# cedricrommel/manipose

Measured on AMD Instinct MI355X. Metric: train poses/sec (whole node), H36M T=243 J=17 K=5, higher is better.
Workload: dtype bf16x3; 1 GPU; H36M lifting T=243 J=17 K=5 ManiPose full (C=512, depth 8), train step fwd+WTA loss+bwd+allreduce+Adam; windows_per_gpu=158, global_batch=158, seq_len=243, parallelism=dp1, precision=bf16x3, gradient_exchange=none

## Files before the change

### manipose_amd/csrc/attention_mfma.hip

```cpp
#include <stdlib.h>
#include "common.h"
#include "kernels.h"

namespace mp {

typedef short bf16x8_t __attribute__((ext_vector_type(8)));
typedef short bf16x4_t __attribute__((ext_vector_type(4)));
typedef float f32x4 __attribute__((ext_vector_type(4)));

constexpr int TP = 256;
constexpr int NTILE = TP / 16;

__device__ __forceinline__ float sfma(float a, float b, float c) { return __builtin_fmaf(a, b, c); }
__device__ __forceinline__ float sadd(float a, float b) {
#pragma clang fp contract(off)
  return a + b;
}
__device__ __forceinline__ float smul(float a, float b) {
#pragma clang fp contract(off)
  return a * b;
}
__device__ __forceinline__ float ssub(float a, float b) {
#pragma clang fp contract(off)
  return a - b;
}

__device__ __forceinline__ float4 bf16x4_to_float4(const uint2& r) {
  return make_float4(__uint_as_float(r.x << 16), __uint_as_float(r.x & 0xffff0000u), __uint_as_float(r.y << 16), __uint_as_float(r.y & 0xffff0000u));
}

template <int D> struct ACfg {
  static constexpr int ROWB = D == 64 ? 128 : 2 * D + 16;
  static __device__ __forceinline__ int swz(int row) { return D == 64 ? (row & 7) : 0; }
  static constexpr int KS = (D + 31) / 32;
  static constexpr int DB = D / 16;
  static constexpr int CH = D / 8;
};

template <int D, int NIMG>
__device__ __forceinline__ void stage_rows_multi(char* const (&S)[NIMG], const bf16* const (&base)[NIMG], const long (&stride)[NIMG], int T, int rows,
                                                 int tid, int nthreads) {
  constexpr int CH = ACfg<D>::CH, ROWB = ACfg<D>::ROWB, U = 2;
  const int total = rows * CH;
  for (int idx0 = tid; idx0 < total; idx0 += U * nthreads) {
    uint4 x[NIMG][U];
#pragma unroll
    for (int u = 0; u < U; ++u) {
      const int idx = min(idx0 + u * nthreads, total - 1);
      const int t = idx / CH, c = idx - t * CH, tc = min(t, T - 1);
#pragma unroll
      for (int im = 0; im < NIMG; ++im) x[im][u] = *reinterpret_cast<const uint4*>(base[im] + (long)tc * stride[im] + c * 8);
    }
#pragma unroll
    for (int u = 0; u < U; ++u) {
      const int idx = idx0 + u * nthreads;
      const int t = idx / CH, c = idx - t * CH;
      if (idx < total) {
#pragma unroll
        for (int im = 0; im < NIMG; ++im)
          *reinterpret_cast<uint4*>(S[im] + t * ROWB + ((c ^ ACfg<D>::swz(t)) << 4)) = (t < T) ? x[im][u] : make_uint4(0u, 0u, 0u, 0u);
      }
    }
  }
}

template <int D> struct ImgRd {
  int fr[ACfg<D>::KS], tc[ACfg<D>::DB];
  bool zero;
  __device__ __forceinline__ void init(const char* img, int lane) {
    constexpr int ROWB = ACfg<D>::ROWB;
    typedef const __attribute__((address_space(3))) char* lds_cptr;
    const int img_off = (int)(unsigned)(size_t)((lds_cptr)img);
    const int l15 = lane & 15, g = lane >> 4, q = l15 >> 2, p = l15 & 3;
    zero = D < 32 && 8 * g >= D;
#pragma unroll
    for (int ks = 0; ks < ACfg<D>::KS; ++ks) {
      fr[ks] = img_off + l15 * ROWB + (((4 * ks + g) ^ ACfg<D>::swz(l15)) << 4);
      asm volatile("" : "+v"(fr[ks]));
    }
#pragma unroll
    for (int db = 0; db < ACfg<D>::DB; ++db) {
      const int row = 4 * g + q;
      tc[db] = img_off + row * ROWB + (((2 * db + (p >> 1)) ^ ACfg<D>::swz(row)) << 4) + (p & 1) * 8;
      asm volatile("" : "+v"(tc[db]));
    }
// ... 731 lines not shown
    if (next < nunits && !MP_ADBG(1)) fetch(next);
    first_unit = false;
    bool q_fetched = false;
    const int h = unit % H, bj = unit / H, j = bj % J, b = bj / J;
#pragma unroll
    for (int sidx = 0; sidx < 2; ++sidx) {
      const int qt = wave + sidx * nw;
      if (qt >= ntile) break;
      const int tq = qt * 16 + l15;
      f32x4 s[NTILE];
      float mx = -INFINITY;
#pragma unroll
      for (int kt = 0; kt < NTILE; ++kt) {
        f32x4 acc = {0.f, 0.f, 0.f, 0.f};
        if (kt < ntile) {
#pragma unroll
          for (int ks = 0; ks < KS; ++ks) {
            const int krow = MP_ADBG(2) ? 0 : kt * 16;
            const bf16x8_t kh = Khr.rows(ks, krow), kl = Khr.rows(ks, krow, dlo);
            if (MP_ADBG(8)) { acc[0] += __builtin_bit_cast(float, (int)kh[0] + (int)kl[1]); continue; }
            MP_MFMA3(acc, kh, kl, qn_h[sidx][ks], qn_l[sidx][ks]);
          }
#pragma unroll
          for (int r = 0; r < 4; ++r) acc[r] = smul(acc[r], scale2);
          if (kt == ntile - 1) {
#pragma unroll
            for (int r = 0; r < 4; ++r)
              if (kt * 16 + 4 * g + r >= T) acc[r] = -INFINITY;
          }
          mx = fmaxf(fmaxf(mx, fmaxf(acc[0], acc[1])), fmaxf(acc[2], acc[3]));
        } else {
          acc = f32x4{-INFINITY, -INFINITY, -INFINITY, -INFINITY};
        }
        s[kt] = acc;
      }
      if (sidx == 1 && next < nunits) { fetch_q(next); q_fetched = true; }
      mx = group_max(mx);
      float sum = 0.f;
#pragma unroll
      for (int kt = 0; kt < NTILE; ++kt) {
        if (MP_ADBG(4)) { sum += s[kt][0]; continue; }
        if (kt < ntile) {
          f32x4 e;
#pragma unroll
          for (int r = 0; r < 4; ++r) e[r] = __builtin_amdgcn_exp2f(ssub(s[kt][r], mx));
          s[kt] = e;
          sum += (e[0] + e[1]) + (e[2] + e[3]);
        } else {
          s[kt] = f32x4{0.f, 0.f, 0.f, 0.f};
        }
      }
      sum = group_sum(sum);
      f32x4 o[DB];
#pragma unroll
      for (int db = 0; db < DB; ++db) o[db] = f32x4{0.f, 0.f, 0.f, 0.f};
#pragma unroll
      for (int kp = 0; kp < NTILE / 2; ++kp) {
        if (2 * kp < ntile) {
          bf16x8_t bph, bpl;
          pack_acc_x2(s[2 * kp], s[2 * kp + 1], bph, bpl);
#pragma unroll
          for (int db = 0; db < DB; ++db) {
            const int vrow = MP_ADBG(2) ? 0 : kp * 32;
            const bf16x8_t vh = Vhr.cols(db, vrow), vl = Vhr.cols(db, vrow, dlo);
            if (MP_ADBG(8)) { o[db][0] += __builtin_bit_cast(float, (int)vh[0] + (int)vl[1] + (int)bph[0] + (int)bpl[0]); continue; }
            MP_MFMA3(o[db], vh, vl, bph, bpl);
          }
        }
      }
      if (tq < T && !(MP_ADBG(16) && sum != 12345.f)) {
        const float inv = 1.0f / sum;
        const long oo = ((long)(b * T + tq) * J + j) * C + h * D;
#pragma unroll
        for (int db = 0; db < DB; ++db) store4_o<F8O>(out_hi + oo + 16 * db + 4 * g, out_lo + oo + 16 * db + 4 * g, o[db], inv);
        if (g == 0) lse[(long)unit * T + tq] = (mx + __log2f(sum)) * 0.6931471805599453f;
      }
    }
    if (next >= nunits) break;
    if (!q_fetched) fetch_q(next);
    unit = next;
  }
}

__device__ __forceinline__ void tm_dma_region(char* __restrict__ region, const bf16* __restrict__ p_hi, const bf16* __restrict__ p_lo, long rs3, int T,
                                              int rows, int lane, int wave, int nw) {
  typedef __attribute__((address_space(3))) void* lptr;
  typedef const __attribute__((address_space(1))) void* gptr;
  const int per_img = rows >> 3;
  for (int n = wave; n < 2 * per_img; n += nw) {
    const int img = n >= per_img, q = n - img * per_img;
    const int r = q * 8 + (lane >> 3), c = (lane & 7) ^ (r & 7);
    const bf16* src = (img ? p_lo : p_hi) + (long)min(r, T - 1) * rs3 + c * 8;
    __builtin_amdgcn_global_load_lds((gptr)src, (lptr)(region + n * 1024), 16, 0, 0);
  }
}

template <bool FULL, bool F8O = false>
__global__ __launch_bounds__(512) void attn_tmfma_fwd_x3p_kernel(const bf16* __restrict__ qkv_hi, const bf16* __restrict__ qkv_lo,
                                                                  bf16* __restrict__ out_hi, bf16* __restrict__ out_lo,
                                                                  float* __restrict__ lse, int nunits, int T, int J, int C, int H, float scale) {
#pragma clang fp contract(off)
  extern __shared__ __attribute__((aligned(16))) char sm[];
  constexpr int D = 64, ROWB = 128, KS = 2, DB = 4, NW = 8, OPITCH = 144;
  const int rows = FULL ? TP : (T + 31) & ~31;
  const int tid = threadIdx.x, lane = tid & 63, g = lane >> 4, l15 = lane & 15;
  const int wave = __builtin_amdgcn_readfirstlane(tid >> 6);
  const long rs3 = (long)J * 3 * C;
  const int ntile = FULL ? NTILE : (T + 15) >> 4;
  const int img_bytes = rows * ROWB;
  char* const regA = sm;
  char* const regB = sm + 2 * img_bytes;
  char* const obuf = sm + 4 * img_bytes + wave * (16 * OPITCH);
  ImgRd<D> Khr, Vhr;
  Khr.init(regA, lane);
  Vhr.init(regB, lane);
  const int dlo = __builtin_amdgcn_readfirstlane(img_bytes);
  const float scale2 = scale * 1.4426950408889634f;
  auto unit_base = [&](int unit) -> long {
    const int h = unit % H, bj = unit / H, j = bj % J, b = bj / J;
    return ((long)b * T * J + j) * 3 * C + h * D;
  };
  bf16x8_t qh[2][KS], ql[2][KS];
  auto fetch_q = [&](int unit) {
    const long qoff = unit_base(unit);
#pragma unroll
    for (int sidx = 0; sidx < 2; ++sidx) {
      const int tq = min((wave + sidx * NW) * 16 + l15, T - 1);
#pragma unroll
      for (int ks = 0; ks < KS; ++ks) {
        qh[sidx][ks] = *reinterpret_cast<const bf16x8_t*>(qkv_hi + qoff + (long)tq * rs3 + 32 * ks + 8 * g);
        ql[sidx][ks] = *reinterpret_cast<const bf16x8_t*>(qkv_lo + qoff + (long)tq * rs3 + 32 * ks + 8 * g);
      }
    }
  };
  int unit = blockIdx.x;
  if (unit >= nunits) return;
  {
    const long qoff = unit_base(unit);
    tm_dma_region(regA, qkv_hi + qoff + C, qkv_lo + qoff + C, rs3, T, rows, lane, wave, NW);
  }
  fetch_q(unit);
  const bool two = wave + NW < ntile;
  while (true) {
    const long qoff = unit_base(unit);
    const int h = unit % H, bj = unit / H, j = bj % J, b = bj / J;
    __builtin_amdgcn_s_waitcnt(0x0070);
    __builtin_amdgcn_s_barrier();
    tm_dma_region(regB, qkv_hi + qoff + 2 * C, qkv_lo + qoff + 2 * C, rs3, T, rows, lane, wave, NW);
    f32x4 s[2][NTILE];
    float mx[2] = {-INFINITY, -INFINITY};
#pragma unroll
    for (int kt = 0; kt < NTILE; ++kt) {
      f32x4 a0 = {0.f, 0.f, 0.f, 0.f}, a1 = {0.f, 0.f, 0.f, 0.f};
      if (kt < ntile) {
#pragma unroll
        for (int ks = 0; ks < KS; ++ks) {
          const bf16x8_t kh = Khr.rows(ks, kt * 16), kl = Khr.rows(ks, kt * 16, dlo);
          MP_MFMA3(a0, kh, kl, qh[0][ks], ql[0][ks]);
          MP_MFMA3(a1, kh, kl, qh[1][ks], ql[1][ks]);
        }
#pragma unroll
        for (int r = 0; r < 4; ++r) { a0[r] = smul(a0[r], scale2); a1[r] = smul(a1[r], scale2); }
        if (kt == ntile - 1) {
#pragma unroll
          for (int r = 0; r < 4; ++r)
            if (kt * 16 + 4 * g + r >= T) { a0[r] = -INFINITY; a1[r] = -INFINITY; }
        }
        mx[0] = fmaxf(fmaxf(mx[0], fmaxf(a0[0], a0[1])), fmaxf(a0[2], a0[3]));
        mx[1] = fmaxf(fmaxf(mx[1], fmaxf(a1[0], a1[1])), fmaxf(a1[2], a1[3]));
      } else {
        a0 = f32x4{-INFINITY, -INFINITY, -INFINITY, -INFINITY};
        a1 = a0;
      }
      s[0][kt] = a0;
      s[1][kt] = a1;
    }
    float sum[2];
#pragma unroll
    for (int sidx = 0; sidx < 2; ++sidx) {
      mx[sidx] = group_max(mx[sidx]);
      float sm_ = 0.f;
#pragma unroll
      for (int kt = 0; kt < NTILE; ++kt) {
        if (kt < ntile) {
          f32x4 e;
#pragma unroll
          for (int r = 0; r < 4; ++r) e[r] = __builtin_amdgcn_exp2f(ssub(s[sidx][kt][r], mx[sidx]));
          s[sidx][kt] = e;
          sm_ += (e[0] + e[1]) + (e[2] + e[3]);
        } else {
          s[sidx][kt] = f32x4{0.f, 0.f, 0.f, 0.f};
        }
      }
      sum[sidx] = group_sum(sm_);
    }
    __builtin_amdgcn_s_waitcnt(0x0070);
    __builtin_amdgcn_s_barrier();
    const int next = unit + gridDim.x;
    if (next < nunits) {
      const long noff = unit_base(next);
      tm_dma_region(regA, qkv_hi + noff + C, qkv_lo + noff + C, rs3, T, rows, lane, wave, NW);
      fetch_q(next);
    }
    f32x4 o[2][DB];
#pragma unroll
    for (int sidx = 0; sidx < 2; ++sidx)
#pragma unroll
      for (int db = 0; db < DB; ++db) o[sidx][db] = f32x4{0.f, 0.f, 0.f, 0.f};
#pragma unroll
    for (int kp = 0; kp < NTILE / 2; ++kp) {
      if (2 * kp < ntile) {
        bf16x8_t p0h, p0l, p1h, p1l;
        pack_acc_x2(s[0][2 * kp], s[0][2 * kp + 1], p0h, p0l);
        pack_acc_x2(s[1][2 * kp], s[1][2 * kp + 1], p1h, p1l);
#pragma unroll
        for (int db = 0; db < DB; ++db) {
          const bf16x8_t vh = Vhr.cols(db, kp * 32), vl = Vhr.cols(db, kp * 32, dlo);
          MP_MFMA3(o[0][db], vh, vl, p0h, p0l);
          MP_MFMA3(o[1][db], vh, vl, p1h, p1l);
        }
      }
    }
#pragma unroll
    for (int sidx = 0; sidx < 2; ++sidx) {
      if (sidx == 1 && !two) break;
      const int qt = wave + sidx * NW;
      const float inv = 1.0f / sum[sidx];
      uint2 hv[DB], lv[DB];
#pragma unroll
      for (int db = 0; db < DB; ++db) {
        if constexpr (F8O) pack4_f16f8(make_float4(o[sidx][db][0] * inv, o[sidx][db][1] * inv, o[sidx][db][2] * inv, o[sidx][db][3] * inv), hv[db], lv[db]);
        else {
          split_bf16x2(o[sidx][db][0] * inv, o[sidx][db][1] * inv, hv[db].x, lv[db].x);
          split_bf16x2(o[sidx][db][2] * inv, o[sidx][db][3] * inv, hv[db].y, lv[db].y);
        }
      }
#pragma unroll
      for (int plane = 0; plane < 2; ++plane) {
#pragma unroll
        for (int db = 0; db < DB; ++db) *reinterpret_cast<uint2*>(obuf + l15 * OPITCH + 32 * db + 8 * g) = plane ? lv[db] : hv[db];
        bf16* const dst = plane ? out_lo : out_hi;
#pragma unroll
        for (int pass = 0; pass < 2; ++pass) {
          const int row = pass * 8 + (lane >> 3), tq = qt * 16 + row;
          const uint4 v = *reinterpret_cast<const uint4*>(obuf + row * OPITCH + (lane & 7) * 16);
          if (tq < T) *reinterpret_cast<uint4*>(dst + ((long)(b * T + tq) * J + j) * C + h * D + (lane & 7) * 8) = v;
        }
      }
      const int tq = qt * 16 + l15;
      if (g == 0 && tq < T) lse[(long)unit * T + tq] = (mx[sidx] + __log2f(sum[sidx])) * 0.6931471805599453f;
    }
    if (next >= nunits) break;
    unit = next;
  }
}

static int g_attn_two_phase = 1;
void attn_two_phase(int on) { g_attn_two_phase = on; }

template <int D, bool F8O = false>
__global__ __launch_bounds__(512) void attn_smfma_fwd_x3_kernel(const bf16* __restrict__ qkv_hi, const bf16* __restrict__ qkv_lo,
                                                                 bf16* __restrict__ out_hi, bf16* __restrict__ out_lo, int nframes, int N, int C,
                                                                 int H, float scale) {
  extern __shared__ __attribute__((aligned(16))) char sm[];
  constexpr int KS = ACfg<D>::KS, DB = ACfg<D>::DB, PER = 7;
  const int tid = threadIdx.x, lane = tid & 63, h = __builtin_amdgcn_readfirstlane(tid >> 6), nthreads = (int)blockDim.x;
  const int g = lane >> 4, l15 = lane & 15;
  const int pitch = 6 * C + 16, cpr = (6 * C) >> 4, nchunk = N * cpr;
  char* sh = sm;
  char* sl = sm + N * pitch;
  uint4 pre[2][PER];
  auto fetch = [&](int f) {
    const char* bh = reinterpret_cast<const char*>(qkv_hi + (long)f * N * 3 * C);
    const char* bl = reinterpret_cast<const char*>(qkv_lo + (long)f * N * 3 * C);
#pragma unroll
    for (int i = 0; i < PER; ++i) {
      const int idx = tid + i * nthreads;
      uint4 a = make_uint4(0u, 0u, 0u, 0u), c = a;
      if (idx < nchunk) { a = *reinterpret_cast<const uint4*>(bh + (long)idx * 16); c = *reinterpret_cast<const uint4*>(bl + (long)idx * 16); }
      pre[0][i] = a; pre[1][i] = c;
    }
  };
  auto commit = [&]() {
#pragma unroll
    for (int i = 0; i < PER; ++i) {
      const int idx = tid + i * nthreads, r = idx / cpr, k = idx - r * cpr;
      if (idx < nchunk) {
        *reinterpret_cast<uint4*>(sh + r * pitch + k * 16) = pre[0][i];
        *reinterpret_cast<uint4*>(sl + r * pitch + k * 16) = pre[1][i];
      }
    }
  };
  const int oq = h * D * 2, ok = 2 * C + oq, ov = 4 * C + oq;
  int f = blockIdx.x;
  if (f >= nframes) return;
  fetch(f);
  while (true) {
    __syncthreads();
    commit();
    __syncthreads();
    const int next = f + gridDim.x;
    if (next < nframes) fetch(next);
    bf16x8_t kfh[2][KS], kfl[2][KS];
#pragma unroll
    for (int t = 0; t < 2; ++t)
#pragma unroll
      for (int ks = 0; ks < KS; ++ks) {
        kfh[t][ks] = frag_tok<D>(sh, pitch, ok, 16 * t, ks, lane, N);
        kfl[t][ks] = frag_tok<D>(sl, pitch, ok, 16 * t, ks, lane, N);
      }
    bf16x8_t vTh[DB], vTl[DB];
#pragma unroll
    for (int db = 0; db < DB; ++db) {
      vTh[db] = frag_tokT<D>(sh, pitch, ov, db, lane, N);
      vTl[db] = frag_tokT<D>(sl, pitch, ov, db, lane, N);
    }
#pragma unroll
    for (int qt = 0; qt < 2; ++qt) {
      if (qt * 16 >= N) break;
      bf16x8_t qfh[KS], qfl[KS];
#pragma unroll
      for (int ks = 0; ks < KS; ++ks) {
        qfh[ks] = frag_tok<D>(sh, pitch, oq, 16 * qt, ks, lane, N);
        qfl[ks] = frag_tok<D>(sl, pitch, oq, 16 * qt, ks, lane, N);
      }
      f32x4 s0 = {0.f, 0.f, 0.f, 0.f}, s1 = {0.f, 0.f, 0.f, 0.f};
#pragma unroll
      for (int ks = 0; ks < KS; ++ks) {
        MP_MFMA3(s0, kfh[0][ks], kfl[0][ks], qfh[ks], qfl[ks]);
        MP_MFMA3(s1, kfh[1][ks], kfl[1][ks], qfh[ks], qfl[ks]);
      }
      col_softmax(s0, s1, g, N, scale);
      bf16x8_t bph, bpl;
      pack_acc_x2(s0, s1, bph, bpl);
      const int tq = qt * 16 + l15;
#pragma unroll
      for (int db = 0; db < DB; ++db) {
        f32x4 o = {0.f, 0.f, 0.f, 0.f};
        MP_MFMA3(o, vTh[db], vTl[db], bph, bpl);
        if (tq < N) {
          const long oo = ((long)f * N + tq) * C + h * D + 16 * db + 4 * g;
          store4_o<F8O>(out_hi + oo, out_lo + oo, o, 1.0f);
// ... 148 lines not shown
      MP_HIP(hipFuncSetAttribute((const void*)attn_tmfma_fwd_x3p_kernel<true>, hipFuncAttributeMaxDynamicSharedMemorySize, (int)(4 * TP * 128 + 8 * 16 * 144)));
      MP_HIP(hipFuncSetAttribute((const void*)attn_tmfma_fwd_x3p_kernel<false, true>, hipFuncAttributeMaxDynamicSharedMemorySize, (int)(4 * TP * 128 + 8 * 16 * 144)));
      MP_HIP(hipFuncSetAttribute((const void*)attn_tmfma_fwd_x3p_kernel<true, true>, hipFuncAttributeMaxDynamicSharedMemorySize, (int)(4 * TP * 128 + 8 * 16 * 144)));
      attr_set = true;
    }
    const int grid = min(units, num_cus());
    const bool full = ((T + 15) >> 4) == NTILE ATTN_X3P_FULL_GUARD;
    if (out_f16f8) {
      if (full) hipLaunchKernelGGL((attn_tmfma_fwd_x3p_kernel<true, true>), dim3(grid), dim3(512), lds, st, qkv_hi, qkv_lo, out_hi, out_lo, lse, units, T, J, C, H, scale);
      else hipLaunchKernelGGL((attn_tmfma_fwd_x3p_kernel<false, true>), dim3(grid), dim3(512), lds, st, qkv_hi, qkv_lo, out_hi, out_lo, lse, units, T, J, C, H, scale);
    } else if (full)
      hipLaunchKernelGGL(attn_tmfma_fwd_x3p_kernel<true>, dim3(grid), dim3(512), lds, st, qkv_hi, qkv_lo, out_hi, out_lo, lse, units, T, J, C, H, scale);
    else
      hipLaunchKernelGGL(attn_tmfma_fwd_x3p_kernel<false>, dim3(grid), dim3(512), lds, st, qkv_hi, qkv_lo, out_hi, out_lo, lse, units, T, J, C, H, scale);
    MP_LAUNCH_CHECK();
    return MP_OK;
  }
  if (D == 64 && out_f16f8) return launch_tmfma_fwd_x3<64, true>(qkv_hi, qkv_lo, out_hi, out_lo, lse, units, T, J, C, H, scale, st);
  if (D == 64) return launch_tmfma_fwd_x3<64>(qkv_hi, qkv_lo, out_hi, out_lo, lse, units, T, J, C, H, scale, st);
  return launch_tmfma_fwd_x3<16>(qkv_hi, qkv_lo, out_hi, out_lo, lse, units, T, J, C, H, scale, st);
}

bool attn_tmfma_supported(int T, int D) { return T <= TP && (D == 64 || D == 16); }

template <int D, int NTC>
static int launch_tmfma_fwd(const bf16* qkv, bf16* out, float* lse, int units, int T, int J, int C, int H, float scale, hipStream_t st) {
  const int ntile = (T + 15) >> 4;
  const int waves = NTC ? 8 : (ntile <= 8 ? (ntile + 1) / 2 : 8);
  const int rows = NTC ? TP : (T + 31) & ~31;
  const size_t lds = 2 * (size_t)rows * ACfg<D>::ROWB;
  static bool attr_set = false;
  if (!attr_set) {
    MP_HIP(hipFuncSetAttribute((const void*)attn_tmfma_fwd_kernel<D, NTC>, hipFuncAttributeMaxDynamicSharedMemorySize,
                               (int)(2 * TP * ACfg<D>::ROWB)));
    attr_set = true;
  }
  hipLaunchKernelGGL((attn_tmfma_fwd_kernel<D, NTC>), dim3(units), dim3(64 * waves), lds, st, qkv, out, lse, T, J, C, H, scale);
  MP_LAUNCH_CHECK();
  return MP_OK;
}
int attn_tmfma_fwd(const bf16* qkv, bf16* out, float* lse, int B, int T, int J, int C, int H, hipStream_t st) {
  const int D = C / H;
  MP_CHECK(attn_tmfma_supported(T, D) && C % 8 == 0, MP_ERR_ARG, "attn_tmfma_fwd: T=%d D=%d unsupported", T, D);
  const float scale = attn_qk_scale(D);
  const int units = B * J * H;
  if (D == 64) return launch_tmfma_fwd<64, 0>(qkv, out, lse, units, T, J, C, H, scale, st);
  return launch_tmfma_fwd<16, 0>(qkv, out, lse, units, T, J, C, H, scale, st);
}

template <int D, int NTC>
static int launch_tmfma_bwd(const bf16* qkv, const bf16* out, const bf16* dout, const float* lse, bf16* dqkv, int units, int T, int J, int C,
                            int H, float scale, int dbg, hipStream_t st, int out_f16) {
  const int ntile = (T + 15) >> 4;
  const int waves = NTC ? 16 : ((ntile >= 5 && ntile <= 7) ? 4 : min(16, ntile));
  const int rows = NTC ? TP : (T + 31) & ~31;
  const size_t lds = 4 * (size_t)rows * ACfg<D>::ROWB + 2 * rows * sizeof(float);
  static bool attr_set = false;
  if (!attr_set) {
    MP_HIP(hipFuncSetAttribute((const void*)attn_tmfma_bwd_kernel<D, NTC, false>, hipFuncAttributeMaxDynamicSharedMemorySize,
                               (int)(4 * TP * ACfg<D>::ROWB + 2 * TP * sizeof(float))));
    MP_HIP(hipFuncSetAttribute((const void*)attn_tmfma_bwd_kernel<D, NTC, true>, hipFuncAttributeMaxDynamicSharedMemorySize,
                               (int)(4 * TP * ACfg<D>::ROWB + 2 * TP * sizeof(float))));
    attr_set = true;
  }
  if (g_grad_f16 != nullptr)
    hipLaunchKernelGGL((attn_tmfma_bwd_kernel<D, NTC, true>), dim3(units), dim3(64 * waves), lds, st, qkv, out, dout, lse, dqkv, T, J, C, H, scale, dbg, g_grad_f16, out_f16);
  else
    hipLaunchKernelGGL((attn_tmfma_bwd_kernel<D, NTC, false>), dim3(units), dim3(64 * waves), lds, st, qkv, out, dout, lse, dqkv, T, J, C, H, scale, dbg, g_grad_f16, out_f16);
  MP_LAUNCH_CHECK();
  return MP_OK;
}
int attn_tmfma_bwd(const bf16* qkv, const bf16* out, const bf16* dout, const float* lse, bf16* dqkv, int B, int T, int J, int C, int H,
                   hipStream_t st, int out_f16) {
  const int D = C / H;
  MP_CHECK(attn_tmfma_supported(T, D) && C % 8 == 0, MP_ERR_ARG, "attn_tmfma_bwd: T=%d D=%d unsupported", T, D);
  const float scale = attn_qk_scale(D);
  const int units = B * J * H;
#ifdef MP_GEMM_DIAG
  static const int dbg = [] { const char* e = getenv("MANIPOSE_ATTN_DEBUG"); return e ? atoi(e) : 0; }();
#else
  constexpr int dbg = 0;
#endif
  const bool full = T > 240;
  if (D == 64) return full ? launch_tmfma_bwd<64, 16>(qkv, out, dout, lse, dqkv, units, T, J, C, H, scale, dbg, st, out_f16)
                           : launch_tmfma_bwd<64, 0>(qkv, out, dout, lse, dqkv, units, T, J, C, H, scale, dbg, st, out_f16);
  return full ? launch_tmfma_bwd<16, 16>(qkv, out, dout, lse, dqkv, units, T, J, C, H, scale, dbg, st, out_f16)
              : launch_tmfma_bwd<16, 0>(qkv, out, dout, lse, dqkv, units, T, J, C, H, scale, dbg, st, out_f16);
}

}
```

### manipose_amd/csrc/capi.hip

```cpp
#include <string.h>
#include "common.h"
#include "kernels.h"
#include "../../include/manipose_hip.h"

namespace mp {
const char* last_error();
long wgrad_f32_slab_floats(int Mtok, int Nout, int Kin);
bool attn_tmfma_supported(int T, int D);
bool attn_smfma_supported(int N, int D, int H);
}
using namespace mp;

static LossCfg to_cfg(const mp_loss_config* c) {
  LossCfg l;
  l.beta = c->rmcl_score_reg; l.vel_w = c->vel_loss; l.smooth_w = c->smooth_reg; l.use_joint_weights = c->w_loss; l.squared = c->sq_loss;
  for (int j = 0; j < 17; ++j) l.joint_weights[j] = c->joint_weights[j];
  return l;
}

extern "C" {

int mp_abi_version(void) { return MP_ABI_VERSION; }
const char* mp_last_error(void) { return mp::last_error(); }

// ... 468 lines not shown
  return ingest_pose2d(raw, raw_joints, raw_channels, frames, (long)N, joint_map, J, res_w, res_h, out, (hipStream_t)stream);
}

int mp_procrustes_errors(const float* pred, const float* gt, const uint8_t* mask, int64_t N, int J, float pred_scale, float gt_scale,
                         float pck_threshold, float auc_max, int auc_steps, float* out, float* scratch, int64_t scratch_floats, void* stream) {
  return procrustes_errors(pred, gt, mask, (long)N, J, pred_scale, gt_scale, pck_threshold, auc_max, auc_steps, 1, out, scratch,
                           (long)scratch_floats, (hipStream_t)stream);
}

int mp_pose_metrics_row_floats(void) { return pose_metrics_row_floats(); }
int mp_bone_length_table(const float* pred, const int64_t* pred_strides, const float* gt, const int64_t* gt_strides, int B, int L, int signed_diff,
                         float* out, void* stream) {
  MP_CHECK(pred && pred_strides && gt && gt_strides && out, MP_ERR_ARG, "mp_bone_length_table: null pointer");
  long ps[4], gs[4];
  for (int i = 0; i < 4; ++i) { ps[i] = (long)pred_strides[i]; gs[i] = (long)gt_strides[i]; }
  return bone_length_table(pred, ps, gt, gs, B, L, signed_diff, out, (hipStream_t)stream);
}
int mp_pose_metrics(const float* pred, const int64_t* pred_strides, const float* gt, const int64_t* gt_strides, const uint8_t* mask, int B,
                    int L, int J, float pred_scale, float gt_scale, float pck_threshold, float auc_max, int auc_steps, int scale_align,
                    float* out, float* len0, float* scratch, int64_t scratch_floats, void* stream) {
  MP_CHECK(pred && pred_strides && out && len0 && scratch, MP_ERR_ARG, "mp_pose_metrics: null pointer");
  long ps[4], gs[4] = {0, 0, 0, 0};
  for (int i = 0; i < 4; ++i) { ps[i] = (long)pred_strides[i]; if (gt_strides) gs[i] = (long)gt_strides[i]; }
  return pose_metrics(pred, ps, gt, gt_strides ? gs : nullptr, mask, B, L, J, pred_scale, gt_scale, pck_threshold, auc_max, auc_steps,
                      scale_align, out, len0, scratch, (long)scratch_floats, (hipStream_t)stream);
}

int64_t mp_bone_extremes_scratch_floats(int64_t frames) { return (int64_t)bone_extremes_scratch_floats((long)frames); }
int mp_bone_extremes(const float* pred, const int64_t* pred_strides, const float* gt, const int64_t* gt_strides, int B, int L, int J,
                     float pred_scale, float gt_scale, int chain, const float* prev_len, int64_t frame_base, float* min_len, float* max_len,
                     float* max_delta, int64_t* max_delta_idx, float* coord_sums, float* last_len, float* scratch, int64_t scratch_floats,
                     void* stream) {
  MP_CHECK(pred && pred_strides, MP_ERR_ARG, "mp_bone_extremes: null pointer");
  long ps[4], gs[4] = {0, 0, 0, 0};
  for (int i = 0; i < 4; ++i) { ps[i] = (long)pred_strides[i]; if (gt_strides) gs[i] = (long)gt_strides[i]; }
  return bone_extremes(pred, ps, gt, gt_strides ? gs : nullptr, B, L, J, pred_scale, gt_scale, chain, prev_len, (long)frame_base, min_len,
                       max_len, max_delta, reinterpret_cast<long*>(max_delta_idx), coord_sums, last_len, scratch, (long)scratch_floats,
                       (hipStream_t)stream);
}

int64_t mp_hypothesis_stats_scratch_floats(int64_t frames) { return (int64_t)hypothesis_stats_scratch_floats((long)frames); }
int mp_hypothesis_stats_row_floats(void) { return hypothesis_stats_row_floats(); }
int mp_hypothesis_stats_row_counts(void) { return hypothesis_stats_row_counts(); }
int mp_hypothesis_stats(const float* poses, const float* scores, const float* target, int B, int K, int T, float pose_scale, float target_scale,
                        float* sums, int64_t* counts, float* jbest_pose, uint8_t* jbest_idx, float* scratch, int64_t scratch_floats,
                        void* stream) {
  return hypothesis_stats(poses, scores, target, B, K, T, pose_scale, target_scale, sums, reinterpret_cast<long*>(counts), jbest_pose, jbest_idx,
                          scratch, (long)scratch_floats, (hipStream_t)stream);
}

int mp_gemm_plan(int M, int N, int K, int form, int epilogue, int cus, int out[4]) {
  MP_CHECK(out, MP_ERR_ARG, "mp_gemm_plan: null out");
  MP_CHECK(M > 0 && N > 0 && K > 0 && cus >= 0, MP_ERR_ARG, "mp_gemm_plan: bad shape M=%d N=%d K=%d cus=%d", M, N, K, cus);
  MP_CHECK(form == GEMM_FORM_BF16 || form == GEMM_FORM_BF16X3 || form == GEMM_FORM_F16F8 || form == GEMM_FORM_F16, MP_ERR_ARG,
           "mp_gemm_plan: form %d (0 bf16, 1 bf16x3, 8 f16f8, 16 fp16)", form);
  MP_CHECK(epilogue >= EPI_BIAS && epilogue <= EPI_SLAB, MP_ERR_ARG, "mp_gemm_plan: epilogue %d", epilogue);
  if (cus == 0) cus = gemm_device_cus();
  MP_CHECK(cus > 0, MP_ERR_HIP, "mp_gemm_plan: no device to ask for its CU count");
  const bool wgrad = epilogue == EPI_SLAB, dgrad = epilogue == EPI_DGELU;
  const GemmPlanIn in = {M, N, K, form, epilogue, wgrad ? 1 : 0, (wgrad || dgrad) ? 1 : 0, 1, wgrad ? (long)M : (long)K, (wgrad || dgrad) ? (long)N : (long)K, 1.0f, cus};
  const GemmPlan pl = gemm_plan(in);
  MP_CHECK(pl.tile != 0, MP_ERR_ARG, "mp_gemm_plan: no kernel of form %d serves M=%d N=%d K=%d with epilogue %d", form, M, N, K, epilogue);
  out[0] = pl.tile; out[1] = pl.persistent; out[2] = pl.workgroups; out[3] = pl.tiles;
  return MP_OK;
}
int mp_gemm_launch_counts(int64_t out[3], int reset) {
  MP_CHECK(out, MP_ERR_ARG, "mp_gemm_launch_counts: null out");
  long long c[3];
  gemm_launch_counts(c, reset);
  for (int i = 0; i < 3; ++i) out[i] = (int64_t)c[i];
  return MP_OK;
}
int mp_set_option(const char* name, int value) {
  MP_CHECK(name, MP_ERR_ARG, "mp_set_option: null name");
  if (!strcmp(name, "gemm_small_tile")) { gemm_bf16_force_small_tile(value != 0); return MP_OK; }
  if (!strcmp(name, "gemm_persist_min_tiles")) { gemm_bf16_persist_min_tiles(value); return MP_OK; }
  if (!strcmp(name, "gemm_persist_mode")) { gemm_bf16_persist_mode(value); return MP_OK; }
  if (!strcmp(name, "gemm_persist_wgs")) { gemm_bf16_persist_wgs(value); return MP_OK; }
  if (!strcmp(name, "gemm_tile")) {
    MP_CHECK(gemm_bf16_tile(value) == MP_OK, MP_ERR_ARG, "mp_set_option: gemm_tile is 0 (planner), 128 or 256, not %d", value);
    return MP_OK;
  }
  if (!strcmp(name, "attn_two_phase")) { attn_two_phase(value); return MP_OK; }
  if (!strcmp(name, "heads_mfma")) { heads_mfma_mode(value); return MP_OK; }
  MP_CHECK(false, MP_ERR_ARG, "mp_set_option: unknown option '%s' (side_streams / f16f8_inputs became mp_model_config::streams / f16f8 in ABI v7)", name);
}

}
```

### manipose_amd/csrc/kernels.h

```cpp
#pragma once
#include "common.h"

namespace mp {

enum { EPI_BIAS = 0, EPI_BIAS_GELU = 1, EPI_BIAS_RESID = 2, EPI_DGELU = 3, EPI_SLAB = 4 };
struct GemmF32Args {
  const float* A;
  const float* B;
  float* C;
  long lda, ldb, ldc;
  int M, N, K;
  const float* bias;
  float* Z;
  const float* R;
  const float* mask;
  float rscale;
  int mask_mode, T, J;
  float* bias_slab;
  int k_per_split;
};
int gemm_f32(int AL, int BL, int EPI, GemmF32Args g, hipStream_t st);
int wgrad_f32(const float* dY, long lddy, const float* X, long ldx, int Mtok, int Nout, int Kin, float* dW, float* db,
              float* slab, long slab_floats, hipStream_t st);

// ... 37 lines not shown
enum { GEMM_FORM_BF16 = 0, GEMM_FORM_BF16X3 = 1, GEMM_FORM_F16F8 = 8, GEMM_FORM_F16 = 16 };
struct GemmPlanIn {
  int M, N, K;
  int form;
  int epi;
  int tra, trb;
  int splits;
  long lda, ldb;
  float rscale;
  int cus;
};
struct GemmPlan {
  int tile;
  int persistent;
  int workgroups;
  int tiles;
};
GemmPlan gemm_plan(const GemmPlanIn& p);
int gemm_device_cus();
int gemm_bf16_tile(int tile);
void gemm_launch_counts(long long out[3], int reset);
void gemm_bf16_force_small_tile(bool on);
void gemm_bf16_persist_min_tiles(int n);
void gemm_bf16_persist_mode(int mode);
void gemm_bf16_persist_wgs(int n);
int gemm_bf16_take_last_persist();

struct LnFwdArgs {
  const float* x;
  int M, C;
  const float* g1; const float* b1; float eps1;
  const float* pos; int T, J;
  float* x1; float* stats1;
  const float* g2; const float* b2; float eps2;
  void* y2; float* stats2;
  void* y2_lo;
  void* y2_b16;
};
int ln_fwd(const LnFwdArgs& a, int out_mode , hipStream_t st);
int ln_bwd(const void* dy, int dy_bf16, const float* x, const float* stats, const float* gamma, const float* dskip, float* dx, void* dx_b16,
           const float* mask, int mask_mode, int T, int J, float* dgamma, float* dbeta, int M, int C, float* scratch,
           long scratch_floats, hipStream_t st, hipStream_t st_param = nullptr, hipEvent_t ev = nullptr, float rs = 1.0f,
           const float* dy_scale = nullptr, const float* b16_gs = nullptr);
int ln_bwd2(const void* dy1, int dy_bf16, const float* x1, const float* stats1, const float* gamma1, const float* dskip,
            const float* x0, const float* stats0, const float* gamma0, const float* beta0 ,
            float* dx, void* dx_b16, const float* mask, int mask_mode, int T, int J, float* dgamma1, float* dbeta1, float* dgamma0, float* dbeta0, int M, int C, float* scratch, long scratch_floats,
            hipStream_t st, hipStream_t st_param = nullptr, hipEvent_t ev = nullptr, float rs = 1.0f, const float* dy_scale = nullptr,
            const float* b16_gs = nullptr);
int grad_scale(const float* d_poses, long n_poses, const float* d_scores, long n_scores, float* gsc, hipStream_t st);
int grad_health_pack(const float* gsc, float* out4, hipStream_t st);
int scale_copy(float* dst, const float* src, float s, long n, hipStream_t st);
int axpy_scaled(float* dst, const float* src, float s, long n, hipStream_t st);

int embed_fwd(const float* xin, const float* W, const float* b, const float* spos, float* out, int M, int C, int J,
              hipStream_t st);
long embed_bwd_scratch_floats(int C, int J);
int embed_bwd(const float* g, const float* xin, float* dW, float* db, float* dspos, int M, int C, int J, float* scratch,
              long scratch_floats, hipStream_t st);
int bones_embed_fwd(const float* xin, const float* W, const float* b, const float* spos, float* out, int BT, int IN, int O,
                    hipStream_t st);
int bones_embed_bwd(const float* g, const float* xin, float* dW, float* db, float* dspos, int BT, int IN, int O,
                    float* scratch, long scratch_floats, hipStream_t st);
int tpos_grad(const float* g, float* dtpos, int B, int T, int J, int C, hipStream_t st);
int scale_rows(const float* g, const float* mask, int mask_mode, void* out, int out_bf16, int M, int C, int T, int J, hipStream_t st);
int adam_step(float* p, const float* g, float* m, float* v, long n, int step, float lr, float beta1, float beta2, float eps,
              float weight_decay, float grad_scale, hipStream_t st, const float* lr_mult = nullptr, const float* wd_mult = nullptr);
struct MaskDesc { int offset, count; float keep; };
int droppath_masks(float* masks, const MaskDesc* descs, int ndesc, unsigned long long seed, unsigned long long step,
                   hipStream_t st);

void attn_grad_f16_override(const float* gout);
void attn_scale_override(float s);
int attn_spatial_fwd(const void* qkv, void* out, int is_bf16, int B, int T, int J, int C, int H, hipStream_t st);
int attn_spatial_bwd(const void* qkv, const void* dout, void* dqkv, int is_bf16, int B, int T, int J, int C, int H, hipStream_t st);
int attn_temporal_fwd(const void* qkv, void* out, float* lse, int is_bf16, int B, int T, int J, int C, int H, hipStream_t st);
int attn_temporal_bwd(const void* qkv, const void* out, const void* dout, const float* lse, float* delta, void* dqkv, int is_bf16,
                      int B, int T, int J, int C, int H, hipStream_t st, int out_f16 = 0);
bool attn_x3_needs_scratch(int temporal, int T, int J, int C, int H);
int attn_spatial_fwd_x3(const bf16* qkv_hi, const bf16* qkv_lo, bf16* out_hi, bf16* out_lo, float* scratch, int B, int T, int J, int C, int H,
                        hipStream_t st, int out_f16f8 = 0);
int attn_temporal_fwd_x3(const bf16* qkv_hi, const bf16* qkv_lo, bf16* out_hi, bf16* out_lo, float* lse, float* scratch, int B, int T, int J,
                         int C, int H, hipStream_t st, int out_f16f8 = 0);
void attn_two_phase(int on);
int join_planes(const bf16* hi, const bf16* lo, float* out, long n, hipStream_t st);
int split_planes(const float* in, bf16* hi, bf16* lo, long n, hipStream_t st);

struct HeadParams { const float* gamma[8]; const float* beta[8]; const float* W[8]; const float* b[8]; };
struct HeadGrads { float* gamma[8]; float* beta[8]; float* W[8]; float* b[8]; };
int heads_fwd(const float* x, const HeadParams& p, int K, int O, float* out, float* stats, int M, int C, hipStream_t st);
bool heads_mfma_supported(int K, int O, int C);
inline long heads_fold_floats(int C) { return 48L * C + 48; }
bool heads_use_mfma(int K, int O, int C);
void heads_mfma_mode(int mode);
int heads_fwd_mfma(const float* x, const HeadParams& p, int K, int O, float* out, float* stats, int M, int C, float* fold, hipStream_t st);
int heads_bwd_mfma(const float* x, const float* stats, const float* fold, const float* out, const HeadParams& p, const HeadGrads& gp, int K, int O,
                   const float* dout, float* dx, int M, int C, float* scratch, long scratch_floats, hipStream_t st, hipStream_t st_param);
int heads_bwd(const float* x, const float* stats, const HeadParams& p, const HeadGrads& gp, int K, int O, const float* dout,
              float* dx, int M, int C, float* scratch, long scratch_floats, hipStream_t st, hipStream_t st_param = nullptr);
struct ScoreParams { const float* w[8]; const float* b[8]; };
struct ScoreGrads { float* w[8]; float* b[8]; };
int scores_fwd(const float* headout, const ScoreParams& p, int K, int O, float* scores, int B, int T, int J, hipStream_t st);
long scores_bwd_scratch_floats(int K, int B, int T);
int scores_bwd(const float* headout, const float* scores, const float* dscores, const ScoreParams& p, const ScoreGrads& gp,
               int K, int O, float* dheadout, int B, int T, int J, float* scratch, long scratch_floats, hipStream_t st, hipStream_t st_param = nullptr, hipEvent_t ev = nullptr);
int bones_mean_fwd(const float* headout, float* lengths, int B, int T, int S, hipStream_t st);
int bones_mean_bwd(const float* dlen_pose, int KT, float* dlengths, float* dheadout, int B, int T, int S, hipStream_t st);

int fk_decode_fwd(const float* rot, int rot_stride, int rot_dim, const float* lengths, float* poses, int B, int K, int T, hipStream_t st);
int fk_decode_bwd(const float* rot, int rot_stride, int rot_dim, const float* lengths, const float* dposes, float* drot,
                  float* dlen_pose, int B, int K, int T, hipStream_t st);

struct LossCfg { float beta, vel_w, smooth_w; int use_joint_weights , squared; float joint_weights[17]; };
int wta_loss(const float* poses, const float* scores, const float* y, const LossCfg& cfg, float* terms, int* argmin,
             float* dposes, float* dscores, int B, int K, int T, float* scratch, long scratch_floats, hipStream_t st);
int single_loss(const float* poses, const float* y, const LossCfg& cfg, float* terms, float* dposes, int B, int T,
                float* scratch, long scratch_floats, hipStream_t st);
int rigid_segments_loss(const float* poses, float weight, float* term, float* dposes, int B, int T, float* scratch, long scratch_floats,
                        hipStream_t st);
int aggregate_poses(const float* poses, const float* scores, const float* y, int mode, float* out, int B, int K, int T,
                    hipStream_t st);
int mpjpe_sum(const float* pred, const float* gt, long njoints, float* out_sum, float* scratch, long scratch_floats,
              hipStream_t st);

int pose_metrics_row_floats();
int bone_length_table(const float* pred, const long* ps, const float* gt, const long* gs, int B, int L, int signed_, float* out, hipStream_t st);
int pose_metrics(const float* pred, const long* ps, const float* gt, const long* gs, const unsigned char* mask, int B, int L, int J,
                 float pred_scale, float gt_scale, float pck_thr, float auc_max, int auc_n, int scale_align, float* out, float* len0,
                 float* scratch, long scratch_floats, hipStream_t st);

long bone_extremes_scratch_floats(long frames);
int bone_extremes(const float* pred, const long* ps, const float* gt, const long* gs, int B, int L, int J, float pred_scale, float gt_scale,
                  int chain, const float* prev_len, long frame_base, float* min_len, float* max_len, float* max_delta, long* max_delta_idx,
                  float* coord_sums, float* last_len, float* scratch, long scratch_floats, hipStream_t st);

long hypothesis_stats_scratch_floats(long frames);
int hypothesis_stats_row_floats();
int hypothesis_stats_row_counts();
int hypothesis_stats(const float* poses, const float* scores, const float* target, int B, int K, int T, float pose_scale, float target_scale,
                     float* sums, long* counts, float* jbest_pose, unsigned char* jbest_idx, float* scratch, long scratch_floats,
                     hipStream_t st);

int gather_windows(const float* p2, const float* p3, const long* seq_offset, int S, const int* win_seq, const int* win_start,
                   const unsigned char* win_flip, const int* mirror, const float* mask2d, const float* noise2d, int B, int T, int J,
                   float* X, float* y, hipStream_t st);

int ingest_pose3d(const float* raw, int Jraw, const int* frames, long N, const int* joint_map, int J, const float* quat,
                  const float* trans, int root_raw, int root_out, float div, float* out, hipStream_t st);
int ingest_pose2d(const float* raw, int Jraw, int Craw, const int* frames, long N, const int* joint_map, int J, float w, float h,
                  float* out, hipStream_t st);

int procrustes_errors(const float* pred, const float* gt, const unsigned char* mask, long N, int J, float pred_scale, float gt_scale,
                      float pck_thr, float auc_max, int auc_n, int scaled, float* out, float* scratch, long scratch_floats, hipStream_t st);

}
```

Measured before the change: 127,100 poses/s.

## Add persistent two-region temporal attention backward kernel with DMA prefetch

```diff
diff --git a/manipose_amd/csrc/attention_mfma.hip b/manipose_amd/csrc/attention_mfma.hip
--- a/manipose_amd/csrc/attention_mfma.hip
+++ b/manipose_amd/csrc/attention_mfma.hip
@@ -1,6 +1,7 @@
 #include <stdlib.h>
 #include "common.h"
 #include "kernels.h"
+#include "attn_dma.h"
 
 namespace mp {
 
@@ -898,17 +899,28 @@
   }
 }
 
+template <typename OffT, bool HIDDEN = false>
+__device__ __forceinline__ void tm_dma_region(char* __restrict__ region, const bf16* __restrict__ p0, const bf16* __restrict__ p1, OffT rb0, OffT rb1, int T,
+                                              int rows, int lane, int wave, int nw) {
+  typedef __attribute__((address_space(3))) void* lptr;
+  typedef const __attribute__((address_space(3))) char* lds_cptr;
+  typedef const __attribute__((address_space(1))) void* gptr;
+  for (int n = wave; n < tm_dma_count(rows); n += nw) {
+    const TmDmaIdx x = tm_dma_index(n, lane, rows, T);
+    const char* src = reinterpret_cast<const char*>(x.img ? p1 : p0) + ((OffT)x.frame * (x.img ? rb1 : rb0) + (OffT)(x.chunk * 16));
+    if constexpr (HIDDEN) {
+      const unsigned dst = (unsigned)(size_t)((lds_cptr)(region + n * TM_DMA_BYTES));
+      unsigned keep;
+      asm volatile("s_mov_b32 %0, m0\n\ts_mov_b32 m0, %2\n\ts_nop 0\n\tglobal_load_lds_dwordx4 %1, off\n\ts_mov_b32 m0, %0"
+                   : "=&s"(keep) : "v"(src), "s"(dst) : "memory");
+    } else {
+      __builtin_amdgcn_global_load_lds((gptr)src, (lptr)(region + n * TM_DMA_BYTES), 16, 0, 0);
+    }
+  }
+}
 __device__ __forceinline__ void tm_dma_region(char* __restrict__ region, const bf16* __restrict__ p_hi, const bf16* __restrict__ p_lo, long rs3, int T,
                                               int rows, int lane, int wave, int nw) {
-  typedef __attribute__((address_space(3))) void* lptr;
-  typedef const __attribute__((address_space(1))) void* gptr;
-  const int per_img = rows >> 3;
-  for (int n = wave; n < 2 * per_img; n += nw) {
-    const int img = n >= per_img, q = n - img * per_img;
-    const int r = q * 8 + (lane >> 3), c = (lane & 7) ^ (r & 7);
-    const bf16* src = (img ? p_lo : p_hi) + (long)min(r, T - 1) * rs3 + c * 8;
-    __builtin_amdgcn_global_load_lds((gptr)src, (lptr)(region + n * 1024), 16, 0, 0);
-  }
+  tm_dma_region<long, true>(region, p_hi, p_lo, 2 * rs3, 2 * rs3, T, rows, lane, wave, nw);
 }
 
 template <bool FULL, bool F8O = false>
@@ -1074,6 +1086,241 @@
 static int g_attn_two_phase = 1;
 void attn_two_phase(int on) { g_attn_two_phase = on; }
 
+template <bool F16G>
+__global__ __launch_bounds__(1024) void attn_tmfma_bwd_p_kernel(const bf16* __restrict__ qkv, const bf16* __restrict__ out,
+                                                                 const bf16* __restrict__ dout, const float* __restrict__ lse,
+                                                                 bf16* __restrict__ dqkv, int nunits, int T, int J, int C, int H, float scale,
+                                                                 const float* __restrict__ gout_p, int out_is_f16) {
+  extern __shared__ __attribute__((aligned(16))) char sm[];
+  constexpr int D = 64, ROWB = ACfg<D>::ROWB, KS = ACfg<D>::KS, DB = ACfg<D>::DB, NW = 16, rows = TP, ntile = NTILE, DQ = D / 16;
+  static_assert(ROWB == TM_DMA_ROWB, "tm_dma_index is written for 128-byte rows");
+  const float gout = F16G ? *gout_p : 0.f;
+  unsigned* const gcnt = F16G ? reinterpret_cast<unsigned*>(const_cast<float*>(gout_p)) + 4 : nullptr;
+  char* const regKV = sm;
+  char* const regQG = sm + 2 * rows * ROWB;
+  float* const stats = reinterpret_cast<float*>(sm + 4 * rows * ROWB);
+  const int tid = threadIdx.x, lane = tid & 63, g = lane >> 4, l15 = lane & 15;
+  const int wave = __builtin_amdgcn_readfirstlane(tid >> 6);
+  const long rs3 = (long)J * 3 * C, rs1 = (long)J * C;
+  auto unit_base = [&](int unit) -> long {
+    const int bj = unit / H, j = bj % J, b = bj / J;
+    return ((long)b * T * J + j) * C;
+  };
+  auto unit_head = [&](int unit) -> int { return (unit % H) * D; };
+  const unsigned rb3 = (unsigned)(rs3 * 2), rb1 = (unsigned)(rs1 * 2);
+  auto here = [](unsigned v) -> unsigned { asm volatile("" : "+v"(v)); return v; };
+  auto strip_row = [&](unsigned l) -> unsigned { return (unsigned)(wave * 16) + (l & 15); };
+  auto at = [&](const bf16* base, unsigned byte_off) -> const char* { return reinterpret_cast<const char*>(base) + byte_off; };
+  constexpr int DH = DQ / 2;
+  auto delta_load = [&](int unit, int half, uint2 (&a)[DH], uint2 (&o)[DH]) {
+    const long ub = unit_base(unit) + unit_head(unit);
+    const unsigned t = here((unsigned)tid), tc = min(t >> 2, (unsigned)(T - 1));
+    const unsigned off = tc * rb1 + (t & 3) * (D / 2);
+#pragma unroll
+    for (int i = 0; i < DH; ++i) {
+      a[i] = *reinterpret_cast<const uint2*>(at(dout + ub + 4 * (half * DH + i), off));
+      o[i] = *reinterpret_cast<const uint2*>(at(out + ub + 4 * (half * DH + i), off));
+    }
+  };
+  auto lse_load = [&](int unit) -> float {
+    const unsigned t = here((unsigned)tid), tc = min(t >> 2, (unsigned)(T - 1));
+    return *reinterpret_cast<const float*>(reinterpret_cast<const char*>(lse + (long)unit * T) + tc * 4);
+  };
+  auto delta_sum = [&](float dl, const uint2 (&a)[DH], const uint2 (&o)[DH]) -> float {
+#pragma unroll
+    for (int i = 0; i < DH; ++i) {
+      const float4 a4 = bf16x4_to_float4(a[i]), o4 = bf16x4_to_float4(out_is_f16 ? f16x4_to_bf16x4(o[i]) : o[i]);
+      dl += (a4.x * o4.x + a4.y * o4.y) + (a4.z * o4.z + a4.w * o4.w);
+    }
+    return dl;
+  };
+  auto delta_commit = [&](float* Ls, float dl, float l) {
+    float* Dl = Ls + rows;
+    const int t = tid >> 2, part = tid & 3;
+    if (t >= T) dl = 0.f;
+    dl += __shfl_xor(dl, 1, 64);
+    dl += __shfl_xor(dl, 2, 64);
+    if (part == 0) {
+      Dl[t] = -dl;
+      Ls[t] = (t < T) ? l * -1.4426950408889634f : -INFINITY;
+    }
+  };
+  bf16x8_t bq[KS], bg[KS];
+  auto fetch_strip = [&](int unit) {
+    const long ub = unit_base(unit);
+    const int hd = unit_head(unit);
+    const unsigned l = here((unsigned)lane), tq = min(strip_row(l), (unsigned)(T - 1));
+    const unsigned o3 = tq * rb3 + 16 * (l >> 4), o1 = tq * rb1 + 16 * (l >> 4);
+#pragma unroll
+    for (int ks = 0; ks < KS; ++ks) {
+      bq[ks] = *reinterpret_cast<const bf16x8_t*>(at(qkv + 3 * ub + hd + 32 * ks, o3));
+      bg[ks] = *reinterpret_cast<const bf16x8_t*>(at(dout + ub + hd + 32 * ks, o1));
+    }
+  };
+  auto dma_kv = [&](int unit) {
+    const bf16* qb = qkv + 3 * unit_base(unit) + unit_head(unit);
+    tm_dma_region<unsigned, true>(regKV, qb + C, qb + 2 * C, rb3, rb3, T, rows, lane, wave, NW);
+  };
+  auto dma_qg = [&](int unit) {
+    const long ub = unit_base(unit);
+    const int hd = unit_head(unit);
+    tm_dma_region<unsigned, true>(regQG, qkv + 3 * ub + hd, dout + ub + hd, rb3, rb1, T, rows, lane, wave, NW);
+  };
+
+  int unit = blockIdx.x;
+  if (unit >= nunits) return;
+  dma_kv(unit);
+  fetch_strip(unit);
+  {
+    uint2 da[DH], dob[DH];
+    float dl = 0.f;
+#pragma unroll
+    for (int half = 0; half < 2; ++half) {
+      delta_load(unit, half, da, dob);
+      dl = delta_sum(dl, da, dob);
+    }
+    delta_commit(stats, dl, lse_load(unit));
+  }
+  const float scale2 = scale * 1.4426950408889634f;
+  int set = 0;
+  while (true) {
+    const float* Ls = stats + set * 2 * rows;
+    const float* Dl = Ls + rows;
+    bf16* const dqu = dqkv + 3 * unit_base(unit) + unit_head(unit);
+    auto dst = [&](bf16* base) -> bf16* {
+      const unsigned l = here((unsigned)lane);
+      return reinterpret_cast<bf16*>(reinterpret_cast<char*>(base) + (strip_row(l) * rb3 + 8 * (l >> 4)));
+    };
+    const int next = unit + gridDim.x;
+    const bool has_next = next < nunits;
+    __builtin_amdgcn_s_waitcnt(0x0070);
+    __builtin_amdgcn_s_barrier();
+    asm volatile("" ::: "memory");
+    dma_qg(unit);
+    uint2 da[DH], dob[DH];
+    float dl_next = 0.f, lse_next = 0.f;
+    if (has_next) delta_load(next, 0, da, dob);
+    bf16x8_t bk[KS], bv[KS];
+
+    {
+      ImgRd<D> Kr, Vr;
+      const int lane_a = (int)here((unsigned)lane);
+      Kr.init(regKV, lane_a);
+      Vr.init(regKV + rows * ROWB, lane_a);
+      const int tq = wave * 16 + l15;
+      const float nL = Ls[tq], ndl = Dl[tq];
+      f32x4 dq[DB];
+#pragma unroll
+      for (int db = 0; db < DB; ++db) dq[db] = f32x4{0.f, 0.f, 0.f, 0.f};
+#pragma unroll
+      for (int kp = 0; kp < ntile / 2; ++kp) {
+        if (kp == ntile / 4 && has_next) {
+          dl_next = delta_sum(dl_next, da, dob);
+          delta_load(next, 1, da, dob);
+          lse_next = lse_load(next);
+        }
+        f32x4 ds[2];
+#pragma unroll
+        for (int hf = 0; hf < 2; ++hf) {
+          const int kt = 2 * kp + hf;
+          f32x4 sc = {0.f, 0.f, 0.f, 0.f}, dp = {0.f, 0.f, 0.f, 0.f};
+#pragma unroll
+          for (int ks = 0; ks < KS; ++ks) {
+            sc = __builtin_amdgcn_mfma_f32_16x16x32_bf16(Kr.rows(ks, kt * 16), bq[ks], sc, 0, 0, 0);
+            dp = __builtin_amdgcn_mfma_f32_16x16x32_bf16(Vr.rows(ks, kt * 16), bg[ks], dp, 0, 0, 0);
+          }
+          f32x4 e;
+#pragma unroll
+          for (int r = 0; r < 4; ++r) e[r] = __builtin_amdgcn_exp2f(sfma(sc[r], scale2, nL));
+          if (kt >= ntile - 1) {
+#pragma unroll
+            for (int r = 0; r < 4; ++r)
+              if (kt * 16 + 4 * g + r >= T) e[r] = 0.f;
+          }
+#pragma unroll
+          for (int r = 0; r < 4; ++r) ds[hf][r] = smul(e[r], sadd(dp[r], ndl));
+        }
+        const bf16x8_t bd = pack_acc(ds[0], ds[1]);
+#pragma unroll
+        for (int db = 0; db < DB; ++db) dq[db] = __builtin_amdgcn_mfma_f32_16x16x32_bf16(Kr.cols(db, kp * 32), bd, dq[db], 0, 0, 0);
+      }
+      if (tq < T) {
+#pragma unroll
+        for (int db = 0; db < DB; ++db) store4g<F16G>(dst(dqu + 16 * db), dq[db], scale, gout, gcnt);
+      }
+#pragma unroll
+      for (int ks = 0; ks < KS; ++ks) {
+        bk[ks] = Kr.rows(ks, wave * 16);
+        bv[ks] = Vr.rows(ks, wave * 16);
+      }
+    }
+    __builtin_amdgcn_sched_barrier(0);
+    if (has_next) {
+      asm volatile("" : "+v"(lse_next));
+      delta_commit(stats + (set ^ 1) * 2 * rows, delta_sum(dl_next, da, dob), lse_next);
+    }
+    __builtin_amdgcn_s_waitcnt(0x0070);
+    __builtin_amdgcn_s_barrier();
+    asm volatile("" ::: "memory");
+    if (has_next) {
+      dma_kv(next);
+      fetch_strip(next);
+    }
+
+    {
+      ImgRd<D> Qr, Gr;
+      const int lane_b = (int)here((unsigned)lane);
+      Qr.init(regQG, lane_b);
+      Gr.init(regQG + rows * ROWB, lane_b);
+      const int tk = wave * 16 + l15;
+      f32x4 dk[DB], dv[DB];
+#pragma unroll
+      for (int db = 0; db < DB; ++db) { dk[db] = f32x4{0.f, 0.f, 0.f, 0.f}; dv[db] = f32x4{0.f, 0.f, 0.f, 0.f}; }
+#pragma unroll
+      for (int qp = 0; qp < ntile / 2; ++qp) {
+        f32x4 p2[2], d2[2];
+#pragma unroll
+        for (int hf = 0; hf < 2; ++hf) {
+          const int qt = 2 * qp + hf;
+          f32x4 sc = {0.f, 0.f, 0.f, 0.f}, dp = {0.f, 0.f, 0.f, 0.f};
+#pragma unroll
+          for (int ks = 0; ks < KS; ++ks) {
+            sc = __builtin_amdgcn_mfma_f32_16x16x32_bf16(Qr.rows(ks, qt * 16), bk[ks], sc, 0, 0, 0);
+            dp = __builtin_amdgcn_mfma_f32_16x16x32_bf16(Gr.rows(ks, qt * 16), bv[ks], dp, 0, 0, 0);
+          }
+          const f32x4 nL = *reinterpret_cast<const f32x4*>(Ls + qt * 16 + 4 * g), ndl = *reinterpret_cast<const f32x4*>(Dl + qt * 16 + 4 * g);
+          f32x4 e;
+#pragma unroll
+          for (int r = 0; r < 4; ++r) e[r] = __builtin_amdgcn_exp2f(sfma(sc[r], scale2, nL[r]));
+          p2[hf] = e;
+#pragma unroll
+          for (int r = 0; r < 4; ++r) d2[hf][r] = smul(e[r], sadd(dp[r], ndl[r]));
+        }
+        const bf16x8_t bp = pack_acc(p2[0], p2[1]), bd = pack_acc(d2[0], d2[1]);
+#pragma unroll
+        for (int db = 0; db < DB; ++db) {
+          dv[db] = __builtin_amdgcn_mfma_f32_16x16x32_bf16(Gr.cols(db, qp * 32), bp, dv[db], 0, 0, 0);
+          dk[db] = __builtin_amdgcn_mfma_f32_16x16x32_bf16(Qr.cols(db, qp * 32), bd, dk[db], 0, 0, 0);
+        }
+      }
+      if (tk < T) {
+#pragma unroll
+        for (int db = 0; db < DB; ++db) {
+          store4g<F16G>(dst(dqu + C + 16 * db), dk[db], scale, gout, gcnt);
+          store4g<F16G>(dst(dqu + 2 * C + 16 * db), dv[db], 1.0f, gout, gcnt);
+        }
+      }
+    }
+    if (!has_next) break;
+    unit = next;
+    set ^= 1;
+  }
+}
+static int g_attn_bwd_two_region = 1;
+static int g_attn_bwd_grid = 0;
+void attn_bwd_two_region(int on) { g_attn_bwd_two_region = on; }
+void attn_bwd_grid(int n) { g_attn_bwd_grid = n; }
+
 template <int D, bool F8O = false>
 __global__ __launch_bounds__(512) void attn_smfma_fwd_x3_kernel(const bf16* __restrict__ qkv_hi, const bf16* __restrict__ qkv_lo,
                                                                  bf16* __restrict__ out_hi, bf16* __restrict__ out_lo, int nframes, int N, int C,
@@ -1388,6 +1635,23 @@
   constexpr int dbg = 0;
 #endif
   const bool full = T > 240;
+  if (D == 64 && full && g_attn_bwd_two_region && (C * 2) % 128 == 0 && (3L * C * 2) % 16 == 0 && (long)T * J * 3 * C * 2 < (1L << 31)) {
+    constexpr size_t lds = 4 * (size_t)TP * 128 + 2 * 2 * TP * sizeof(float);
+    static bool attr_set = false;
+    if (!attr_set) {
+      MP_HIP(hipFuncSetAttribute((const void*)attn_tmfma_bwd_p_kernel<false>, hipFuncAttributeMaxDynamicSharedMemorySize, (int)lds));
+      MP_HIP(hipFuncSetAttribute((const void*)attn_tmfma_bwd_p_kernel<true>, hipFuncAttributeMaxDynamicSharedMemorySize, (int)lds));
+      attr_set = true;
+    }
+    int grid = min(units, num_cus());
+    if (g_attn_bwd_grid > 0) grid = min(grid, g_attn_bwd_grid);
+    if (g_grad_f16 != nullptr)
+      hipLaunchKernelGGL(attn_tmfma_bwd_p_kernel<true>, dim3(grid), dim3(1024), lds, st, qkv, out, dout, lse, dqkv, units, T, J, C, H, scale, g_grad_f16, out_f16);
+    else
+      hipLaunchKernelGGL(attn_tmfma_bwd_p_kernel<false>, dim3(grid), dim3(1024), lds, st, qkv, out, dout, lse, dqkv, units, T, J, C, H, scale, g_grad_f16, out_f16);
+    MP_LAUNCH_CHECK();
+    return MP_OK;
+  }
   if (D == 64) return full ? launch_tmfma_bwd<64, 16>(qkv, out, dout, lse, dqkv, units, T, J, C, H, scale, dbg, st, out_f16)
                            : launch_tmfma_bwd<64, 0>(qkv, out, dout, lse, dqkv, units, T, J, C, H, scale, dbg, st, out_f16);
   return full ? launch_tmfma_bwd<16, 16>(qkv, out, dout, lse, dqkv, units, T, J, C, H, scale, dbg, st, out_f16)
diff --git a/manipose_amd/csrc/attn_dma.h b/manipose_amd/csrc/attn_dma.h
--- /dev/null
+++ b/manipose_amd/csrc/attn_dma.h
@@ -0,0 +1,35 @@
+#pragma once
+
+#if defined(__HIPCC__) || defined(__CUDACC__)
+#define MP_ATTN_HD __host__ __device__
+#else
+#define MP_ATTN_HD
+#endif
+
+namespace mp {
+
+constexpr int TM_DMA_ROWB = 128;
+constexpr int TM_DMA_BYTES = 1024;
+
+struct TmDmaIdx {
+  int img;
+  int lds;
+  int frame;
+  int chunk;
+};
+
+MP_ATTN_HD inline int tm_dma_count(int rows) { return 2 * (rows >> 3); }
+
+MP_ATTN_HD inline TmDmaIdx tm_dma_index(int n, int lane, int rows, int T) {
+  const int per_img = rows >> 3;
+  const int img = n >= per_img, q = n - img * per_img;
+  const int r = q * 8 + (lane >> 3);
+  TmDmaIdx x;
+  x.img = img;
+  x.lds = n * TM_DMA_BYTES + lane * 16;
+  x.frame = r < T - 1 ? r : T - 1;
+  x.chunk = (lane & 7) ^ (r & 7);
+  return x;
+}
+
+}
diff --git a/manipose_amd/csrc/capi.hip b/manipose_amd/csrc/capi.hip
--- a/manipose_amd/csrc/capi.hip
+++ b/manipose_amd/csrc/capi.hip
@@ -574,6 +574,12 @@
     return MP_OK;
   }
   if (!strcmp(name, "attn_two_phase")) { attn_two_phase(value); return MP_OK; }
+  if (!strcmp(name, "attn_bwd_two_region")) { attn_bwd_two_region(value != 0); return MP_OK; }
+  if (!strcmp(name, "attn_bwd_grid")) {
+    MP_CHECK(value >= 0, MP_ERR_ARG, "mp_set_option: attn_bwd_grid is 0 (one workgroup per CU) or a workgroup count, not %d", value);
+    attn_bwd_grid(value);
+    return MP_OK;
+  }
   if (!strcmp(name, "heads_mfma")) { heads_mfma_mode(value); return MP_OK; }
   MP_CHECK(false, MP_ERR_ARG, "mp_set_option: unknown option '%s' (side_streams / f16f8_inputs became mp_model_config::streams / f16f8 in ABI v7)", name);
 }
diff --git a/manipose_amd/csrc/kernels.h b/manipose_amd/csrc/kernels.h
--- a/manipose_amd/csrc/kernels.h
+++ b/manipose_amd/csrc/kernels.h
@@ -143,6 +143,8 @@
 int attn_temporal_fwd_x3(const bf16* qkv_hi, const bf16* qkv_lo, bf16* out_hi, bf16* out_lo, float* lse, float* scratch, int B, int T, int J,
                          int C, int H, hipStream_t st, int out_f16f8 = 0);
 void attn_two_phase(int on);
+void attn_bwd_two_region(int on);
+void attn_bwd_grid(int n);
 int join_planes(const bf16* hi, const bf16* lo, float* out, long n, hipStream_t st);
 int split_planes(const float* in, bf16* hi, bf16* lo, long n, hipStream_t st);
 
```

Result: no change. 127,200 poses/s (median of 2 runs) (+0.0%).
